# VictoriaMetrics/VictoriaLogs

Measured on NVIDIA H100. Metric: log rows scanned/sec (LogsQL phrase+regex), higher is better.
Workload: dtype u8

## Files before the change

victorialogs_b200/csrc/vl_zstd.cu:

```cuda
#include "vl_zstd.h"

#include <algorithm>
#include <array>
#include <atomic>
#include <chrono>
#include <cstdio>
#include <cstdlib>
#include <cstring>
#include <exception>
#include <thread>

#include "vl_engine.h"
#include "vl_zstd.cuh"
#include "vl_zstd_job.h"

namespace vl {

using namespace zs;

struct ZstdDev {
    DevBuf frames, blocks, bstate, huf_tab, fse_tab, huf_state, fse_state, predef, lits, seqs, frame_err, status, lists;
    bool predef_ready = false;
    cudaStream_t xstream = nullptr;
    std::vector<cudaEvent_t> events;
// ... 78 lines not shown
    auto taper = [&] { if (!group_scale_env()) m->limit_scale = (m->groups.empty() || m->n_seqs > total_seqs - total_seqs / 12) ? 1 : 4; };
    for (size_t i = 0; i < n; i++) {
        try {
            uint32_t f1 = 0, f2 = 0;
            taper();
            const size_t c1 = add_bytes_block(v[i].p, v[i].n, v[i].zoff, &info[i].lens_len, &f1);
            taper();
            const size_t c2 = add_bytes_block(v[i].p + c1, v[i].n - c1, v[i].zoff + c1, &info[i].data_len, &f2);
            if (c1 + c2 != v[i].n) throw BadInput("unexpected non-empty tail after reading bytes block with strings");
        } catch (const BadInput& e) { *bad = i; *msg = e.msg; return; }
    }
    if (!group_scale_env()) m->limit_scale = 1;
}

void ZstdJob::prepare() { m->prepare(); }

void ZstdJob::digest(uint64_t out[4]) const { m->digest(out); }

void ZstdJob::run(vlscan_ctx* ctx, const uint8_t* zsrc, uint8_t* arena) {
    Impl& J = *m;
    if (J.frames.empty()) return;
    auto now = [] { return std::chrono::duration<double>(std::chrono::steady_clock::now().time_since_epoch()).count(); };
    const double t_prep = now();
    J.prepare();
    const double t_lists = now();
    const std::vector<uint32_t>& lists = J.lists;
    if (!ctx->zdev) ctx->zdev = new ZstdDev;
    ZstdDev& D = *ctx->zdev;
    cudaStream_t st = ctx->stream;
    D.frames.ensure(J.frames.size() * sizeof(ZFrame) + 16); D.blocks.ensure(J.blocks.size() * sizeof(ZBlock) + 16); D.bstate.ensure(J.blocks.size() * sizeof(ZBlockState));
    D.frame_err.ensure(J.frames.size() * 4); D.status.ensure(16); D.lists.ensure(lists.size() * 4 + 16);
    D.huf_tab.ensure(std::max<size_t>((size_t)J.max_huf * Z_HUF_TABLE * 2, 16)); D.huf_state.ensure(std::max<size_t>((size_t)J.max_huf * sizeof(ZSlotState), 16));
    D.fse_tab.ensure(std::max<size_t>((size_t)J.max_fse * Z_FSE_SLOT_BYTES, 16)); D.fse_state.ensure(std::max<size_t>((size_t)J.max_fse * sizeof(ZSlotState), 16));
    const size_t lits_stride = (J.max_lits + 64 + 255) / 256 * 256, seqs_stride = std::max<size_t>(J.max_seqs, 1);
    D.lits.ensure(2 * lits_stride); D.seqs.ensure(2 * seqs_stride * 16);
    if (!D.xstream) VL_CUDA(cudaStreamCreateWithFlags(&D.xstream, cudaStreamNonBlocking));
    if (!D.predef_ready) {
        D.predef.ensure(Z_FSE_SLOT_BYTES);
        k_zstd_predef<<<1, 32, 0, st>>>(D.predef.as<uint8_t>());
        VL_CUDA(cudaFuncSetAttribute(k_seq_decode, cudaFuncAttributeMaxDynamicSharedMemorySize, (int)(Z_SEQ_CTA_LANES * (Z_FSE_SLOT_BYTES + Z_LINEBUF))));
        VL_CUDA(cudaFuncSetAttribute(k_huf_decode, cudaFuncAttributeMaxDynamicSharedMemorySize, (int)(Z_HUF_CTA_BLOCKS * Z_HUF_TABLE * 2)));
        ctx->launches++; VL_CUDA(cudaGetLastError());
        D.predef_ready = true;
    }
    {
        auto up16 = [](size_t n) { return (n + 15) / 16 * 16; };
        const size_t nf = up16(J.frames.size() * sizeof(ZFrame)), nb = up16(J.blocks.size() * sizeof(ZBlock)), nl = up16(lists.size() * 4);
        uint8_t* h = (uint8_t*)D.ensure_hpin(nf + nb + nl + 64);
        const double t_cp = now();
        J.spread_copy(h, J.frames.data(), J.frames.size() * sizeof(ZFrame));
        J.spread_copy(h + nf, J.blocks.data(), J.blocks.size() * sizeof(ZBlock));
        if (!lists.empty()) J.spread_copy(h + nf + nb, lists.data(), lists.size() * 4);
        if (getenv("VLSCAN_DEBUG_TIMING")) fprintf(stderr, "[vlscan zstd] host: work lists of %zu launch groups %.1f ms, %.1f MB of tables to pinned memory %.1f ms (%d threads)\n",
                                                   J.groups.size(), 1e3 * (t_lists - t_prep), (nf + nb + nl) / 1e6, 1e3 * (now() - t_cp), std::max(J.threads, 1));
        k_pull_words<<<296, 256, 0, st>>>(D.frames.as<uint4>(), (const uint4*)h, nf / 16); ctx->launches++;
        k_pull_words<<<296, 256, 0, st>>>(D.blocks.as<uint4>(), (const uint4*)(h + nf), nb / 16); ctx->launches++;
        if (nl) { k_pull_words<<<296, 256, 0, st>>>(D.lists.as<uint4>(), (const uint4*)(h + nf + nb), nl / 16); ctx->launches++; }
        VL_CUDA(cudaGetLastError());
    }
    VL_CUDA(cudaMemsetAsync(D.frame_err.p, 0, J.frames.size() * 4, st));
    VL_CUDA(cudaMemsetAsync(D.status.p, 0, 16, st));
    VL_CUDA(cudaMemsetAsync(D.bstate.p, 0, J.blocks.size() * sizeof(ZBlockState), st));
    ZView V{};
    V.src = zsrc; V.arena = arena; V.frames = D.frames.as<ZFrame>(); V.blocks = D.blocks.as<ZBlock>(); V.bstate = D.bstate.as<ZBlockState>();
    V.huf_tab = D.huf_tab.as<uint16_t>(); V.fse_tab = D.fse_tab.as<uint8_t>(); V.huf_state = D.huf_state.as<ZSlotState>(); V.fse_state = D.fse_state.as<ZSlotState>();
    V.predef = D.predef.as<uint8_t>(); V.lits = D.lits.as<uint8_t>(); V.seqs = D.seqs.as<uint4>(); V.frame_err = D.frame_err.as<unsigned int>();
    V.status = D.status.as<unsigned long long>();
    const uint32_t* L = D.lists.as<uint32_t>();
    const bool dbg = getenv("VLSCAN_DEBUG_TIMING") != nullptr;
    static const char* phase_name[6] = {"huf_build", "huf_decode", "fse_build", "seq_decode", "seq_resolve", "execute"};
    std::vector<std::pair<int, std::pair<cudaEvent_t, cudaEvent_t>>> marks;
    int phase = 0;
    static const bool overlap = [] { const char* e = getenv("VLSCAN_ZSTD_OVERLAP"); return !e || atoi(e) != 0; }();
    cudaStream_t xs = overlap ? D.xstream : st;
    cudaStream_t cur_stream = st;
    auto begin = [&](int p) { phase = p; if (dbg) { cudaEvent_t a, b; cudaEventCreate(&a); cudaEventCreate(&b); cudaEventRecord(a, cur_stream); marks.push_back({p, {a, b}}); } };
    auto launched = [&] { ctx->launches++; VL_CUDA(cudaGetLastError()); if (dbg) cudaEventRecord(marks.back().second.second, cur_stream); };
    VL_CUDA(cudaEventRecord(D.event(0), st)); VL_CUDA(cudaStreamWaitEvent(xs, D.event(0), 0));
    size_t gi = 0;
    for (const Group& g : J.groups) {
        uint32_t nh = g.huf_hi - g.huf_lo, nl = g.lit_hi - g.lit_lo, ns = g.seq_hi - g.seq_lo, nf = g.frame_hi - g.frame_lo;
        if (J.group_hook) {
            uint64_t need = 0;
            for (uint32_t i = J.frames[g.frame_lo].blk_lo; i < J.frames[g.frame_hi - 1].blk_hi; i++) need = std::max<uint64_t>(need, J.blocks[i].src + (J.blocks[i].type == ZB_RLE ? 1 : J.blocks[i].size));
            J.group_hook(need);
        }
        ZView W = V;
        W.lits = V.lits + (gi & 1) * lits_stride; W.seqs = V.seqs + (gi & 1) * seqs_stride;
        cudaEvent_t ev_entropy = D.event(1 + 2 * gi), ev_exec = D.event(2 + 2 * gi);
        cur_stream = st;
        if (gi >= 2) VL_CUDA(cudaStreamWaitEvent(st, D.event(2 + 2 * (gi - 2)), 0));
        if (nh) { begin(0); k_huf_build<<<cdiv_u(nh, 4), 128, 0, st>>>(W, L + g.huf_lo, nh); launched(); }
        if (nl) { begin(1); k_huf_decode<<<cdiv_u(nl, Z_HUF_CTA_BLOCKS), Z_HUF_CTA_BLOCKS * 4, Z_HUF_CTA_BLOCKS * Z_HUF_TABLE * 2, st>>>(W, L + g.lit_lo, nl); launched(); }
        if (ns) {
            begin(2); k_fse_build<<<cdiv_u(ns, 64), 64, 0, st>>>(W, L + g.seq_lo, ns); launched();
            begin(3); k_seq_decode<<<cdiv_u(ns, Z_SEQ_CTA_LANES), 64, Z_SEQ_CTA_LANES * (Z_FSE_SLOT_BYTES + Z_LINEBUF), st>>>(W, L + g.seq_lo, ns); launched();
        }
        VL_CUDA(cudaEventRecord(ev_entropy, st));
        VL_CUDA(cudaStreamWaitEvent(xs, ev_entropy, 0));
        cur_stream = xs;
        begin(4); k_seq_resolve<<<cdiv_u(nf, 64), 64, 0, xs>>>(W, g.frame_lo, nf); launched();
        begin(5); k_execute<<<cdiv_u((uint64_t)nf * 32, Z_EXEC_WARPS * 32), Z_EXEC_WARPS * 32, 0, xs>>>(W, L + g.ord_lo, nf); launched();
        VL_CUDA(cudaEventRecord(ev_exec, xs));
        gi++;
    }
    if (gi) VL_CUDA(cudaStreamWaitEvent(st, D.event(2 + 2 * (gi - 1)), 0));
    cur_stream = st;
    if (dbg) {
        VL_CUDA(cudaStreamSynchronize(xs)); VL_CUDA(cudaStreamSynchronize(st));
        float tot[6] = {0, 0, 0, 0, 0, 0};
        for (auto& mk : marks) { float ms = 0; cudaEventElapsedTime(&ms, mk.second.first, mk.second.second); tot[mk.first] += ms; cudaEventDestroy(mk.second.first); cudaEventDestroy(mk.second.second); }
        fprintf(stderr, "[vlscan zstd] %zu groups:", J.groups.size());
        for (int p = 0; p < 6; p++) fprintf(stderr, " %s %.2f ms", phase_name[p], tot[p]);
        fprintf(stderr, "\n");
    }
    (void)phase;
    J.ran = true;
}

void ZstdJob::check(vlscan_ctx* ctx) {
    if (!m->ran) return;
    unsigned long long stt[2] = {0, 0};
    VL_CUDA(cudaMemcpyAsync(stt, ctx->zdev->status.p, 16, cudaMemcpyDeviceToHost, ctx->stream));
    VL_CUDA(cudaStreamSynchronize(ctx->stream));
    if (!stt[0]) return;
    static const char* what[] = {"", "bad Huffman tree description", "bad Huffman stream", "bad FSE table description", "bad sequences bitstream", "match offset beyond the regenerated data",
                                 "regenerated size differs from the frame content size", "bad literals section"};
    throw BadInput(std::string("cannot decompress block: ") + (stt[0] < 8 ? what[stt[0]] : "corrupted frame") + " (frame " + std::to_string(stt[1] - 1) + " of the batch)");
}

}
```

victorialogs_b200/csrc/vl_zstd.cuh:

```cuda
#pragma once
#include <cuda_runtime.h>
#include <stdint.h>
#include "vl_zstd_types.h"

namespace vl {
namespace zs {

struct ZView {
    const uint8_t* src;
    uint8_t* arena;
    const ZFrame* frames; const ZBlock* blocks; ZBlockState* bstate;
    uint16_t* huf_tab; uint8_t* fse_tab; ZSlotState* huf_state; ZSlotState* fse_state;
    const uint8_t* predef;
    uint8_t* lits; uint4* seqs;
    unsigned int* frame_err;
    unsigned long long* status;
};

static __device__ __forceinline__ void zfail(const ZView& V, uint32_t frame, unsigned code) {
    atomicCAS(&V.frame_err[frame], 0u, code);
    atomicMax(&V.status[0], (unsigned long long)code);
    atomicMax(&V.status[1], (unsigned long long)frame + 1);
}

static __device__ __forceinline__ uint64_t ldu64(const uint8_t* p) {
    uintptr_t a = (uintptr_t)p & ~(uintptr_t)7; uint32_t sh = (uint32_t)((uintptr_t)p & 7) * 8;
    uint64_t lo = *(const uint64_t*)a;
    if (!sh) return lo;
    uint64_t hi = *(const uint64_t*)(a + 8);
    return (lo >> sh) | (hi << (64 - sh));
}
static __device__ __forceinline__ uint64_t peek64(const uint8_t* base, int64_t pos) {
    if (pos >= 64) { int junk = (int)((-pos) & 7); return ldu64(base + ((pos + 7) >> 3) - 8) << junk; }
    if (pos <= 0) return 0;
    uint64_t v = 0; int nb = (int)((pos + 7) >> 3);
    for (int i = 0; i < nb; i++) v |= (uint64_t)base[i] << (8 * i);
    return v << (64 - pos);
}
struct BackReader {
    const uint8_t* base; int64_t pos; uint64_t w; int avail;
    __device__ __forceinline__ bool init(const uint8_t* p, uint32_t len) {
        base = p; w = 0; avail = 0; pos = 0;
        if (!len) return false;
        uint32_t last = p[len - 1];
        if (!last) return false;
        pos = (int64_t)len * 8 - (int64_t)(__clz(last) - 23);
        return true;
// ... 155 lines not shown
            for (int i = 0; i < nw; i++) { if (w[i] > 11) { ok = 0; break; } if (w[i]) sum += 1u << (w[i] - 1); }
            if (ok && sum == 0) ok = 0;
            if (ok) {
                maxbits = hibit(sum) + 1;
                uint32_t left = (1u << maxbits) - sum;
                if (maxbits > 11 || (left & (left - 1)) != 0) ok = 0;
                else { w[nw++] = (uint8_t)(hibit(left) + 1); }
            }
        }
        if (ok) {
            uint32_t cnt[13]; for (int i = 0; i < 13; i++) cnt[i] = 0;
            for (int i = 0; i < nw; i++) cnt[w[i]]++;
            uint32_t nxt[13]; uint32_t acc = 0;
            for (int k = 1; k <= maxbits; k++) { nxt[k] = acc; acc += cnt[k] << (k - 1); }
            for (int i = 0; i < nw; i++) if (w[i]) { s_start[wi][i] = (uint16_t)nxt[w[i]]; nxt[w[i]] += 1u << (w[i] - 1); }
        }
        s_meta[wi][0] = nw; s_meta[wi][1] = maxbits; s_meta[wi][2] = ok;
        V.bstate[bi].huf_desc_len = desc;
    }
    __syncwarp();
    if (!s_meta[wi][2]) { if (lane == 0) zfail(V, B.frame, ZERR_HUF_DESC); return; }
    const int nw = s_meta[wi][0], maxbits = s_meta[wi][1];
    uint16_t* tab = V.huf_tab + (size_t)B.huf_own * Z_HUF_TABLE;
    for (int s = (int)lane; s < nw; s += 32) {
        uint32_t ww = w[s];
        if (!ww) continue;
        uint32_t len = 1u << (ww - 1), st = s_start[wi][s];
        uint16_t e = (uint16_t)(s | ((maxbits + 1 - ww) << 8));
        for (uint32_t k = 0; k < len; k++) tab[st + k] = e;
    }
    if (lane == 0) V.huf_state[B.huf_own].huf_maxbits = (uint8_t)maxbits;
}

static const uint32_t Z_HUF_CTA_BLOCKS = 56;
static __global__ void __launch_bounds__(Z_HUF_CTA_BLOCKS * 4) k_huf_decode(ZView V, const uint32_t* __restrict__ list, uint32_t n) {
    extern __shared__ uint16_t s_tab[];
    const uint32_t local = threadIdx.x >> 2, k = threadIdx.x & 3;
    const uint32_t first = blockIdx.x * Z_HUF_CTA_BLOCKS;
    const uint32_t here = min(Z_HUF_CTA_BLOCKS, n - first);
    for (uint32_t it = 0; it < here; it++) {
        const ZBlock& Bt = V.blocks[list[first + it]];
        const uint32_t entries = 1u << V.huf_state[Bt.huf_slot].huf_maxbits;
        const uint4* g = (const uint4*)(V.huf_tab + (size_t)Bt.huf_slot * Z_HUF_TABLE);
        uint4* d = (uint4*)(s_tab + (size_t)it * Z_HUF_TABLE);
        for (uint32_t e = threadIdx.x; e < entries / 8; e += blockDim.x) d[e] = g[e];
        if (entries < 8 && threadIdx.x == 0) d[0] = g[0];
    }
    __syncthreads();
    if (local >= here) return;
    const uint32_t bi = list[first + local];
    const ZBlock& B = V.blocks[bi];
    if (V.frame_err[B.frame]) return;
    if (B.lit_streams == 1 && k) return;
    const uint32_t maxbits = V.huf_state[B.huf_slot].huf_maxbits;
    const uint16_t* tab = s_tab + (size_t)local * Z_HUF_TABLE;
    const uint32_t desc = B.lit_type == ZL_COMPRESSED ? V.bstate[bi].huf_desc_len : 0;
    if (maxbits == 0 || desc > B.lit_comp) { zfail(V, B.frame, ZERR_HUF_STREAM); return; }
    const uint8_t* s = V.src + B.src + B.lit_hdr + desc;
    uint32_t total = B.lit_comp - desc, len, nout;
    uint8_t* out = V.lits + B.lit_off;
    if (B.lit_streams == 1) { len = total; nout = B.lit_regen; }
    else {
        if (total < 6) { if (!k) zfail(V, B.frame, ZERR_HUF_STREAM); return; }
        uint32_t s1 = s[0] | (s[1] << 8), s2 = s[2] | (s[3] << 8), s3 = s[4] | (s[5] << 8);
        if ((uint64_t)6 + s1 + s2 + s3 > total) { if (!k) zfail(V, B.frame, ZERR_HUF_STREAM); return; }
        uint32_t seg = (B.lit_regen + 3) / 4;
        if (3 * seg > B.lit_regen) { if (!k) zfail(V, B.frame, ZERR_HUF_STREAM); return; }
// ... 47 lines not shown
    if (t >= n) return;
    const uint32_t bi = list[t];
    const ZBlock& B = V.blocks[bi];
    const uint8_t* p = V.src + B.src;
    uint32_t off = B.seq_hdr + 1;
    bool ok = off <= B.size && (B.modes & 3) == 0;
    int16_t freq[53]; uint16_t nx[53];
    ZSlotState st{0, 0, 0, 0};
    for (int k = 0; k < 3 && ok; k++) {
        int mode = k == 0 ? (B.modes >> 6) & 3 : k == 1 ? (B.modes >> 4) & 3 : (B.modes >> 2) & 3;
        int max_al = k == 1 ? 8 : 9, max_syms = k == 0 ? 36 : k == 1 ? 32 : 53;
        uint32_t toff = k == 0 ? Z_FSE_LL : k == 1 ? Z_FSE_OF : Z_FSE_ML;
        int al = 0;
        if (mode == 1) {
            if (off + 1 > B.size) { ok = false; break; }
            uint32_t sym = p[off++];
            if ((int)sym >= max_syms) { ok = false; break; }
            uint8_t* slot = V.fse_tab + (size_t)B.fse_own * Z_FSE_SLOT_BYTES;
            ((uint16_t*)slot)[toff] = 0; slot[2 * Z_FSE_ENTRIES + toff] = (uint8_t)sym;
        } else if (mode == 2) {
            int ns = 0;
            uint32_t used = off < B.size ? fse_read_counts(p + off, B.size - off, max_al, max_syms, freq, &ns, &al) : 0;
            uint8_t* slot = V.fse_tab + (size_t)B.fse_own * Z_FSE_SLOT_BYTES;
            if (!used || !fse_build_seq_table((uint16_t*)slot + toff, slot + 2 * Z_FSE_ENTRIES + toff, al, freq, ns, nx)) { ok = false; break; }
            off += used;
        } else continue;
        if (k == 0) st.ll_al = (uint8_t)al; else if (k == 1) st.of_al = (uint8_t)al; else st.ml_al = (uint8_t)al;
    }
    if (!ok || off > B.size) { zfail(V, B.frame, ZERR_FSE_DESC); return; }
    if (B.fse_own != Z_PREDEF) V.fse_state[B.fse_own] = st;
    V.bstate[bi].seq_bits_off = off;
}

static const uint32_t Z_SEQ_CTA_LANES = 56;
static const uint32_t Z_LINEBUF = 272;
static const uint32_t Z_SEQ_LEAD = 160;
static __device__ __forceinline__ uint32_t lds_u32(uint32_t sa) { uint32_t v; asm volatile("ld.shared.u32 %0, [%1];" : "=r"(v) : "r"(sa)); return v; }
static __device__ __forceinline__ uint32_t bfe_u32(uint32_t a, uint32_t pos, uint32_t len) { uint32_t d; asm("bfe.u32 %0, %1, %2, %3;" : "=r"(d) : "r"(a), "r"(pos), "r"(len)); return d; }
static __device__ __forceinline__ uint32_t top_bits(uint32_t x, uint32_t n) { return __funnelshift_rc(x, 0u, 32u - n); }
struct SeqLane {
    const uint8_t* gorg;
    uint32_t ring;
    uint32_t p;
    uint32_t fc;
    const uint16_t* tr; const uint8_t* sy; const uint32_t* llv; const uint32_t* mlv;
    uint32_t sl, so, sm, r1, r2, r3, ndirty, sum_ll, sum_ml, sticky;
    uint4* out;
    __device__ __forceinline__ void fetch_chunk() {
        fc--;
        const uint32_t sa = ring + ((fc & 15u) << 4);
        const uint8_t* g = gorg + (size_t)fc * 16;
        asm volatile("cp.async.cg.shared.global [%0], [%1], 16;" ::"r"(sa), "l"(g) : "memory");
    }
    __device__ __forceinline__ void window(uint32_t& c2, uint32_t& c1, uint32_t& c0) const {
        const uint32_t k = (p - 1u) >> 5, s = (0u - p) & 31u;
        const uint32_t w3 = lds_u32(ring + ((k << 2) & 252u)), w2 = lds_u32(ring + (((k - 1u) << 2) & 252u));
        const uint32_t w1 = lds_u32(ring + (((k - 2u) << 2) & 252u)), w0 = lds_u32(ring + (((k - 3u) << 2) & 252u));
        c2 = __funnelshift_l(w2, w3, s); c1 = __funnelshift_l(w1, w2, s); c0 = __funnelshift_l(w0, w1, s);
    }
    template <bool LAST>
    __device__ __forceinline__ void step() {
        const uint32_t tl = tr[sl], to = tr[so], tm = tr[sm];
        const uint32_t oc = sy[so], vl = llv[sy[sl]], vm = mlv[sy[sm]];
        if (p < fc * 128u + Z_SEQ_LEAD * 8u && fc > 0) fetch_chunk();
        asm volatile("cp.async.commit_group;\n\tcp.async.wait_group 3;" ::: "memory");
        uint32_t c2, c1, c0;
        window(c2, c1, c0);
        const uint32_t nL = vl >> 24, nM = vm >> 24, n2 = nM + nL;
        const uint32_t ov = (1u << oc) + top_bits(c2, oc);
        const uint32_t v2 = top_bits(__funnelshift_l(c1, c2, oc), n2);
        const uint32_t ml = (vm & 0xFFFFFFu) + (v2 >> nL), ll = (vl & 0xFFFFFFu) + bfe_u32(v2, 0, nL);
        const uint32_t o3 = oc + n2;
        if (!LAST) {
            const uint32_t bL = tl >> 12, bM = tm >> 12, bO = to >> 12, n3 = bL + bM + bO;
            const bool up = o3 < 32;
            const uint32_t v3 = top_bits(__funnelshift_l(up ? c1 : c0, up ? c2 : c1, o3), n3);
            sl = Z_FSE_LL + (tl & 0xFFFu) + (v3 >> (bM + bO));
            sm = Z_FSE_ML + (tm & 0xFFFu) + bfe_u32(v3, bO, bM);
            so = Z_FSE_OF + (to & 0xFFFu) + bfe_u32(v3, 0, bO);
            p -= o3 + n3;
        } else p -= o3;
        uint32_t o;
        if (ov > 3) { o = ov - 3; r3 = r2; r2 = r1; r1 = o; }
        else {
            const uint32_t idx = ov + (ll == 0 ? 1 : 0);
            if (idx == 1) o = r1;
            else {
                o = idx == 2 ? r2 : idx == 3 ? r3 : (r1 == 0xFFFFFFFFu ? r1 : r1 - 1);
                if (idx != 2) r3 = r2;
                r2 = r1; r1 = o;
            }
        }
        ndirty += (r1 | r2 | r3) >> 31;
        *out++ = make_uint4(ll, ml, o, ov);
        sum_ll += ll; sum_ml += ml;
        sticky |= p | sum_ll | sum_ml;
    }
};
static __global__ void __launch_bounds__(64) k_seq_decode(ZView V, const uint32_t* __restrict__ list, uint32_t n) {
    extern __shared__ __align__(16) uint8_t s_fse[];
    __shared__ uint32_t s_llv[36], s_mlv[53];
    const uint32_t first = blockIdx.x * Z_SEQ_CTA_LANES;
    const uint32_t here = min(Z_SEQ_CTA_LANES, n - first);
    if (threadIdx.x < 36) s_llv[threadIdx.x] = Z_LL_BASE[threadIdx.x] | ((uint32_t)Z_LL_BITS[threadIdx.x] << 24);
    if (threadIdx.x < 53) s_mlv[threadIdx.x] = Z_ML_BASE[threadIdx.x] | ((uint32_t)Z_ML_BITS[threadIdx.x] << 24);
    for (uint32_t it = 0; it < here; it++) {
        const ZBlock& Bt = V.blocks[list[first + it]];
        const uint4* src_ll = (const uint4*)(Bt.ll_slot == Z_PREDEF ? V.predef : V.fse_tab + (size_t)Bt.ll_slot * Z_FSE_SLOT_BYTES);
        const uint4* src_ml = (const uint4*)(Bt.ml_slot == Z_PREDEF ? V.predef : V.fse_tab + (size_t)Bt.ml_slot * Z_FSE_SLOT_BYTES);
        const uint4* src_of = (const uint4*)(Bt.of_slot == Z_PREDEF ? V.predef : V.fse_tab + (size_t)Bt.of_slot * Z_FSE_SLOT_BYTES);
        uint4* d = (uint4*)(s_fse + (size_t)it * Z_FSE_SLOT_BYTES);
        for (uint32_t c = threadIdx.x; c < Z_FSE_SLOT_BYTES / 16; c += blockDim.x) {
            const uint4* src = c < 64 ? src_ll : c < 128 ? src_ml : c < 160 ? src_of : c < 192 ? src_ll : c < 224 ? src_ml : src_of;
            d[c] = src[c];
        }
    }
    __syncthreads();
    if (threadIdx.x >= here) return;
    const uint32_t bi = list[first + threadIdx.x];
    const ZBlock& B = V.blocks[bi];
    if (V.frame_err[B.frame]) return;
    const uint32_t off = V.bstate[bi].seq_bits_off;
    const int ll_al = B.ll_slot == Z_PREDEF ? 6 : V.fse_state[B.ll_slot].ll_al;
    const int of_al = B.of_slot == Z_PREDEF ? 5 : V.fse_state[B.of_slot].of_al;
    const int ml_al = B.ml_slot == Z_PREDEF ? 6 : V.fse_state[B.ml_slot].ml_al;
    if (off >= B.size) { zfail(V, B.frame, ZERR_SEQ_STREAM); return; }
    const uint64_t st = B.src + off;
    const uint32_t len = B.size - off;
    const uint32_t last = V.src[st + len - 1];
    if (!last) { zfail(V, B.frame, ZERR_SEQ_STREAM); return; }
    SeqLane L;
    const uint64_t org = (st & ~255ull) - 256;
    const uint32_t s0 = (uint32_t)(st - org) * 8;
    L.gorg = V.src + org;
    L.ring = (uint32_t)__cvta_generic_to_shared(s_fse + (size_t)Z_SEQ_CTA_LANES * Z_FSE_SLOT_BYTES + (size_t)threadIdx.x * Z_LINEBUF);
    L.p = s0 + len * 8 - (uint32_t)(__clz(last) - 23);
    L.fc = ((L.p - 1u) >> 7) + 1u;
#pragma unroll
    for (int q = 0; q < 12; q++) L.fetch_chunk();
    asm volatile("cp.async.commit_group;\n\tcp.async.wait_group 0;" ::: "memory");
    L.tr = (const uint16_t*)(s_fse + (size_t)threadIdx.x * Z_FSE_SLOT_BYTES);
    L.sy = s_fse + (size_t)threadIdx.x * Z_FSE_SLOT_BYTES + 2 * Z_FSE_ENTRIES;
    L.llv = s_llv; L.mlv = s_mlv;
    {
        uint32_t c2, c1, c0;
        L.window(c2, c1, c0);
        L.sl = Z_FSE_LL + top_bits(c2, ll_al);
        L.so = Z_FSE_OF + top_bits(__funnelshift_l(c1, c2, ll_al), of_al);
        L.sm = Z_FSE_ML + top_bits(__funnelshift_l(c1, c2, ll_al + of_al), ml_al);
        L.p -= ll_al + of_al + ml_al;
        (void)c0;
    }
    const uint32_t DIRTY = 0xFFFFFFFFu;
    L.r1 = B.rep_known ? 1 : DIRTY; L.r2 = B.rep_known ? 4 : DIRTY; L.r3 = B.rep_known ? 8 : DIRTY;
    L.ndirty = 0; L.sum_ll = 0; L.sum_ml = 0; L.sticky = L.p;
    L.out = V.seqs + B.seq_base;
    const uint32_t nseq = B.nseq;
    for (uint32_t i = 0; i + 1 < nseq; i++) L.step<false>();
    if (nseq) L.step<true>();
    asm volatile("cp.async.wait_group 0;" ::: "memory");
    if ((L.sticky >> 31) || L.p != s0 || L.sum_ll > B.lit_regen) { zfail(V, B.frame, ZERR_SEQ_STREAM); return; }
    ZBlockState& S = V.bstate[bi];
    S.out_len = B.lit_regen + L.sum_ml;
    S.clean_from = B.rep_known ? 0 : L.ndirty + 1;
    S.rep[0] = L.r1; S.rep[1] = L.r2; S.rep[2] = L.r3;
}

static __global__ void __launch_bounds__(64) k_seq_resolve(ZView V, uint32_t frame_lo, uint32_t nframes) {
    const uint32_t t = blockIdx.x * blockDim.x + threadIdx.x;
    if (t >= nframes) return;
    const uint32_t f = frame_lo + t;
    if (V.frame_err[f]) return;
    const ZFrame& F = V.frames[f];
    uint64_t out = 0;
    uint32_t r1 = 1, r2 = 4, r3 = 8;
    for (uint32_t bi = F.blk_lo; bi < F.blk_hi; bi++) {
        const ZBlock& B = V.blocks[bi];
        ZBlockState& S = V.bstate[bi];
        S.out_base = (uint32_t)out;
        if (B.type != ZB_COMPRESSED) { out += B.size; S.out_len = B.size; continue; }
        if (!B.nseq) { S.out_len = B.lit_regen; out += B.lit_regen; }
        else {
            uint4* __restrict__ sq = V.seqs + B.seq_base;
            const uint32_t redo = min(S.clean_from, B.nseq);
            for (uint32_t i = 0; i < redo; i++) {
                uint4 q = sq[i];
                uint32_t ll = q.x, ov = q.w, o;
                if (ov > 3) { o = ov - 3; r3 = r2; r2 = r1; r1 = o; }
                else {
                    uint32_t idx = ov + (ll == 0 ? 1 : 0);
                    if (idx == 1) o = r1;
                    else {
                        o = idx == 2 ? r2 : idx == 3 ? r3 : r1 - 1;
                        if (idx != 2) r3 = r2;
                        r2 = r1; r1 = o;
                    }
                }
                sq[i].z = o;
            }
            if (S.clean_from <= B.nseq) { r1 = S.rep[0]; r2 = S.rep[1]; r3 = S.rep[2]; }
            out += S.out_len;
        }
        if (out > F.fcs) { zfail(V, f, ZERR_SIZE); return; }
    }
    if (out != F.fcs) zfail(V, f, ZERR_SIZE);
}

static const uint32_t Z_RING = 4096;
static const uint32_t Z_EXEC_WARPS = 4;
static __device__ __forceinline__ uint32_t ldu32(const uint8_t* p) {
    const uintptr_t a = (uintptr_t)p & ~(uintptr_t)3;
    const uint32_t lo = *(const uint32_t*)a, hi = *(const uint32_t*)(a + 4);
    return __funnelshift_r(lo, hi, (uint32_t)((uintptr_t)p & 3) * 8);
}
static __global__ void __launch_bounds__(128) k_execute(ZView V, const uint32_t* __restrict__ order, uint32_t nframes) {
    __shared__ __align__(16) uint8_t s_ring[Z_EXEC_WARPS][Z_RING];
    const uint32_t wid = (blockIdx.x * blockDim.x + threadIdx.x) >> 5, lane = threadIdx.x & 31;
    if (wid >= nframes) return;
    const uint32_t f = order[wid];
    if (V.frame_err[f]) return;
    const ZFrame& F = V.frames[f];
    uint8_t* dst = V.arena + F.dst;
    uint8_t* ring = s_ring[threadIdx.x >> 5];
    const uint32_t abase = (uint32_t)(uintptr_t)dst;
#define VL_RIDX(p) ((abase + (p)) & (Z_RING - 1))
#define VL_RING(p) ring[VL_RIDX(p)]
    uint32_t ring_lo = 0;
    for (uint32_t bi = F.blk_lo; bi < F.blk_hi; bi++) {
        const ZBlock& B = V.blocks[bi];
        const uint32_t blk_base = V.bstate[bi].out_base;
        const uint8_t* p = V.src + B.src;
        if (B.type == ZB_RAW) { for (uint32_t k = lane; k < B.size; k += 32) { uint8_t v = p[k]; dst[blk_base + k] = v; VL_RING(blk_base + k) = v; } __syncwarp(); continue; }
        if (B.type == ZB_RLE) { uint8_t v = p[0]; for (uint32_t k = lane; k < B.size; k += 32) { dst[blk_base + k] = v; VL_RING(blk_base + k) = v; } __syncwarp(); continue; }
        const uint8_t* lit = B.lit_type == ZL_RAW ? p + B.lit_hdr : V.lits + B.lit_off;
        const bool lit_rle = B.lit_type == ZL_RLE;
        const uint8_t rle_byte = lit_rle ? p[B.lit_hdr] : 0;
        const uint4* __restrict__ sq = V.seqs + B.seq_base;
        uint32_t lit_run = 0, out_run = blk_base;
        uint4 qn = lane < B.nseq ? sq[lane] : make_uint4(0, 0, 0, 0);
        for (uint32_t g = 0; g < B.nseq; g += 32) {
            const uint4 q = qn;
            qn = g + 32 + lane < B.nseq ? sq[g + 32 + lane] : make_uint4(0, 0, 0, 0);
            uint32_t il = q.x, io = q.x + q.y;
#pragma unroll
            for (int d = 1; d < 32; d <<= 1) { uint32_t a = __shfl_up_sync(0xffffffffu, il, d), b = __shfl_up_sync(0xffffffffu, io, d); if ((int)lane >= d) { il += a; io += b; } }
            const uint32_t lit_start = il - q.x;
            const uint32_t o_start = io - q.x - q.y;
            const uint32_t T = __shfl_sync(0xffffffffu, il, 31), O = __shfl_sync(0xffffffffu, io, 31);
            const uint32_t gend = out_run + O;
            const uint32_t cnt = min(32u, B.nseq - g);
            const uint32_t ml = q.y, off = q.z, amd = out_run + o_start + q.x;
            if (__any_sync(0xffffffffu, lane < cnt && (off == 0 || off > amd))) { if (lane == 0) zfail(V, f, ZERR_OFFSET); return; }
            const uint32_t s_src = amd - off, e_src = s_src + min(ml, off);
            int dep = -1;
            {
                uint32_t lo = 0;
#pragma unroll
                for (int s = 16; s; s >>= 1) { uint32_t v = __shfl_sync(0xffffffffu, amd, (lo + s - 1) & 31); if ((lo + s - 1) < cnt && v < e_src) lo += s; }
                const uint32_t ci = (lo - 1) & 31;
                const uint32_t ca = __shfl_sync(0xffffffffu, amd, ci), cm = __shfl_sync(0xffffffffu, ml, ci);
                if (lo > 0 && ca + cm > s_src) dep = (int)lo - 1;
            }
            if (O < Z_RING) {
                uint32_t cl = (q.x + 3) >> 2, cm = (ml + 3) >> 2;
#pragma unroll
                for (int d = 1; d < 32; d <<= 1) { uint32_t a = __shfl_up_sync(0xffffffffu, cl, d), b = __shfl_up_sync(0xffffffffu, cm, d); if ((int)lane >= d) { cl += a; cm += b; } }
                const uint32_t CL = __shfl_sync(0xffffffffu, cl, 31);
                const uint32_t pk = lit_start | (o_start << 16);
                const uint8_t* lsrc = lit + lit_run;
                for (uint32_t c0 = 0; c0 < CL; c0 += 128) {
                    uint32_t w[4], at[4], nb[4];
#pragma unroll
                    for (int u = 0; u < 4; u++) {
                        nb[u] = 0; w[u] = 0; at[u] = 0;
                        if (c0 + 32 * u >= CL) continue;
// ... 124 lines not shown
```

victorialogs_b200/csrc/vl_zstd_job.h:

```cpp
#pragma once
#include <stddef.h>
#include <stdint.h>
#include <stdlib.h>
#include <string.h>
#include <algorithm>
#include <array>
#include <atomic>
#include <exception>
#include <functional>
#include <string>
#include <thread>
#include <vector>
#include "vl_zstd.h"
#include "vl_zstd_types.h"
#include "vl_zstd_walk.h"

namespace vl {

using namespace zs;

inline uint64_t group_scale_env() { static const uint64_t v = [] { const char* e = getenv("VLSCAN_ZSTD_GROUP_SCALE"); long x = e ? atol(e) : 0; return (uint64_t)(x < 0 ? 0 : x > 64 ? 64 : x); }(); return v; }
static const uint64_t kGroupLitsUnit = 512ull << 20, kGroupSeqsUnit = 64ull << 20;
static const uint32_t kGroupSlotsUnit = 32u << 10;

struct Group { uint32_t frame_lo, frame_hi; uint32_t huf_lo, huf_hi, lit_lo, lit_hi, seq_lo, seq_hi, ord_lo, ord_hi; };

struct FrameUse { uint64_t lits, seqs; uint32_t huf, fse; };

struct ZstdJobImpl {
    std::vector<ZFrame> frames;
    std::vector<ZBlock> blocks;
    std::vector<Group> groups;
    std::vector<uint32_t> lists;
    uint64_t g_lits = 0, g_seqs = 0; uint32_t g_huf = 0, g_fse = 0; uint32_t g_frame_lo = 0;
    uint64_t limit_scale = group_scale_env() ? group_scale_env() : 4;
    uint64_t max_lits = 0, max_seqs = 0; uint32_t max_huf = 0, max_fse = 0;
    uint64_t n_compressed = 0, n_seqs = 0;
    int threads = 0;
    bool prepared = false, ran = false;
    std::function<void(uint64_t)> group_hook;

    void close_group_at(uint32_t f) {
        if (g_frame_lo == f) return;
        Group g{}; g.frame_lo = g_frame_lo; g.frame_hi = f;
        groups.push_back(g);
        max_lits = std::max(max_lits, g_lits); max_seqs = std::max(max_seqs, g_seqs); max_huf = std::max(max_huf, g_huf); max_fse = std::max(max_fse, g_fse);
        g_lits = g_seqs = 0; g_huf = g_fse = 0; g_frame_lo = f;
    }
    void close_group() { close_group_at((uint32_t)frames.size()); }

    static FrameUse frame_use(const ZBlock* b, uint32_t cnt) {
        FrameUse u{0, 0, 0, 0};
        for (uint32_t i = 0; i < cnt; i++) {
            if (b[i].type != ZB_COMPRESSED) continue;
            if (b[i].lit_type >= ZL_COMPRESSED) u.lits += b[i].lit_regen;
            u.seqs += b[i].nseq; u.huf += b[i].huf_own != Z_PREDEF; u.fse += b[i].fse_own != Z_PREDEF;
        }
        return u;
    }
    FrameUse admit_frame(uint32_t f, const FrameUse& u) {
        const uint64_t m = limit_scale;
        if (g_frame_lo != f && (g_lits + u.lits > kGroupLitsUnit * m || g_seqs + u.seqs > kGroupSeqsUnit * m || g_huf + u.huf > kGroupSlotsUnit * m || g_fse + u.fse > kGroupSlotsUnit * m)) close_group_at(f);
        FrameUse base{g_lits, g_seqs, g_huf, g_fse};
        g_lits += u.lits; g_seqs += u.seqs; g_huf += u.huf; g_fse += u.fse;
        return base;
    }
    static void place_blocks(ZBlock* b, uint32_t cnt, FrameUse base, uint64_t& n_compressed, uint64_t& n_seqs) {
        for (uint32_t i = 0; i < cnt; i++) {
            ZBlock& B = b[i];
            if (B.type != ZB_COMPRESSED) continue;
// ... 85 lines not shown
        const size_t G = groups.size();
        std::vector<std::vector<uint32_t>> gl(G);
        std::vector<std::array<uint32_t, 4>> cnt(G);
        std::atomic<size_t> next{0};
        const int T = (int)std::max<size_t>(1, std::min<size_t>((size_t)std::max(threads, 1), G));
        on_threads(T, [&](int) {
            std::vector<std::pair<uint32_t, uint32_t>> v; std::vector<uint32_t> count;
            for (;;) {
                const size_t gi = next.fetch_add(1);
                if (gi >= G) return;
                const Group& g = groups[gi];
                std::vector<uint32_t>& L = gl[gi];
                const uint32_t blo = frames[g.frame_lo].blk_lo, bhi = frames[g.frame_hi - 1].blk_hi;
                auto by_desc = [&] {
                    uint32_t kmax = 0; for (auto& e : v) kmax = std::max(kmax, e.first);
                    if (v.size() >= 64 && kmax < (1u << 16)) {
                        count.assign((size_t)kmax + 2, 0);
                        for (auto& e : v) count[kmax - e.first + 1]++;
                        for (uint32_t k = 0; k <= kmax; k++) count[k + 1] += count[k];
                        const size_t at = L.size(); L.resize(at + v.size());
                        for (auto& e : v) L[at + count[kmax - e.first]++] = e.second;
                    } else {
                        std::stable_sort(v.begin(), v.end(), [](const auto& a, const auto& b) { return a.first > b.first; });
                        for (auto& e : v) L.push_back(e.second);
                    }
                    v.clear();
                };
                for (uint32_t i = blo; i < bhi; i++) if (blocks[i].type == ZB_COMPRESSED && blocks[i].lit_type == ZL_COMPRESSED) L.push_back(i);
                cnt[gi][0] = (uint32_t)L.size();
                for (uint32_t i = blo; i < bhi; i++) if (blocks[i].type == ZB_COMPRESSED && blocks[i].lit_type >= ZL_COMPRESSED) v.push_back({blocks[i].lit_regen >> 9, i});
                by_desc(); cnt[gi][1] = (uint32_t)L.size();
                for (uint32_t i = blo; i < bhi; i++) if (blocks[i].type == ZB_COMPRESSED && blocks[i].nseq) v.push_back({blocks[i].nseq >> 6, i});
                by_desc(); cnt[gi][2] = (uint32_t)L.size();
                for (uint32_t i = g.frame_lo; i < g.frame_hi; i++) v.push_back({(uint32_t)(frames[i].fcs >> 10), i});
                by_desc(); cnt[gi][3] = (uint32_t)L.size();
            }
        });
        size_t total = 0; for (auto& L : gl) total += L.size();
        if (total > 0xFFFFFFF0ull) throw BadInput("too many ZSTD blocks in one batch");
        lists.resize(total);
        size_t off = 0;
        for (size_t gi = 0; gi < G; gi++) {
            Group& g = groups[gi];
            g.huf_lo = (uint32_t)off; g.huf_hi = g.lit_lo = (uint32_t)(off + cnt[gi][0]); g.lit_hi = g.seq_lo = (uint32_t)(off + cnt[gi][1]);
            g.seq_hi = g.ord_lo = (uint32_t)(off + cnt[gi][2]); g.ord_hi = (uint32_t)(off + cnt[gi][3]);
            if (!gl[gi].empty()) memcpy(lists.data() + off, gl[gi].data(), gl[gi].size() * 4);
            off += gl[gi].size();
        }
    }

    void spread_copy(void* dst, const void* src, size_t n) const {
        const int T = (int)std::max<size_t>(1, std::min<size_t>((size_t)std::max(threads, 1), n / (4u << 20) + 1));
        on_threads(T, [&](int t) { const size_t lo = n * (size_t)t / (size_t)T, hi = n * (size_t)(t + 1) / (size_t)T; if (hi > lo) memcpy((uint8_t*)dst + lo, (const uint8_t*)src + lo, hi - lo); });
    }

    void digest(uint64_t out[4]) const {
        const ZstdJobImpl& J = *this;
        auto mix = [](uint64_t& h, uint64_t v) { h = (h ^ v) * 0x9E3779B97F4A7C15ull; h ^= h >> 29; };
        uint64_t h0 = 1, h1 = 2, h2 = 3, h3 = 4;
        for (const ZFrame& f : J.frames) { mix(h0, f.dst); mix(h0, f.fcs); mix(h0, ((uint64_t)f.blk_lo << 32) | f.blk_hi); }
        for (const ZBlock& b : J.blocks) {
            mix(h1, b.src); mix(h1, b.lit_off); mix(h1, b.seq_base); mix(h1, ((uint64_t)b.size << 32) | b.frame); mix(h1, ((uint64_t)b.lit_hdr << 32) | b.lit_regen);
            mix(h1, ((uint64_t)b.lit_comp << 32) | b.nseq); mix(h1, ((uint64_t)b.seq_hdr << 32) | b.huf_slot); mix(h1, ((uint64_t)b.huf_own << 32) | b.fse_own);
            mix(h1, ((uint64_t)b.ll_slot << 32) | b.of_slot); mix(h1, ((uint64_t)b.ml_slot << 32) | ((uint64_t)b.type << 24) | ((uint64_t)b.lit_type << 16) | ((uint64_t)b.lit_streams << 8) | b.modes); mix(h1, b.rep_known);
        }
        for (const Group& g : J.groups) for (uint32_t x : {g.frame_lo, g.frame_hi, g.huf_lo, g.huf_hi, g.lit_lo, g.lit_hi, g.seq_lo, g.seq_hi, g.ord_lo, g.ord_hi}) mix(h2, x);
        for (uint64_t x : {J.max_lits, J.max_seqs, (uint64_t)J.max_huf, (uint64_t)J.max_fse, J.n_compressed, J.n_seqs, (uint64_t)J.groups.size()}) mix(h2, x);
        for (uint32_t x : J.lists) mix(h3, x);
        out[0] = h0; out[1] = h1; out[2] = h2; out[3] = h3;
    }
};

}
```

victorialogs_b200/csrc/vl_zstd_types.h:

```cpp
#pragma once
#include <stdint.h>

namespace vl {
namespace zs {

enum { ZERR_NONE = 0, ZERR_HUF_DESC = 1, ZERR_HUF_STREAM = 2, ZERR_FSE_DESC = 3, ZERR_SEQ_STREAM = 4, ZERR_OFFSET = 5, ZERR_SIZE = 6, ZERR_LITERALS = 7 };
enum { ZB_RAW = 0, ZB_RLE = 1, ZB_COMPRESSED = 2 };
enum { ZL_RAW = 0, ZL_RLE = 1, ZL_COMPRESSED = 2, ZL_TREELESS = 3 };
static const uint32_t Z_PREDEF = 0xFFFFFFFFu;
static const uint32_t Z_HUF_TABLE = 2048;
static const uint32_t Z_FSE_LL = 0, Z_FSE_ML = 512, Z_FSE_OF = 1024, Z_FSE_ENTRIES = 1280, Z_FSE_SLOT_BYTES = 3 * 1280;

struct ZFrame {
    uint64_t dst;
    uint64_t fcs;
    uint32_t blk_lo, blk_hi;
};
struct ZBlock {
    uint64_t src;
    uint64_t lit_off;
    uint64_t seq_base;
    uint32_t size;
    uint32_t frame;
    uint32_t lit_hdr;
    uint32_t lit_regen, lit_comp;
    uint32_t nseq;
    uint32_t seq_hdr;
    uint32_t huf_slot;
    uint32_t huf_own;
    uint32_t fse_own;
    uint32_t ll_slot, of_slot, ml_slot;
    uint8_t type, lit_type, lit_streams, modes;
    uint8_t rep_known;
    uint8_t pad[3];
};
struct ZBlockState {
    uint32_t huf_desc_len;
    uint32_t seq_bits_off;
    uint32_t out_len;
    uint32_t out_base;
    uint32_t clean_from;
    uint32_t rep[3];
};
struct ZSlotState { uint8_t huf_maxbits, ll_al, of_al, ml_al; };
// ... 4 lines not shown
```

Measured before the change: 21.35 billion.

## Pack decoded zstd sequences into 64-bit words and shrink seq/huf CTA sizes

Decoded sequences are stored as packed 64-bit words (18-bit literal and match lengths, a 2-bit repeat code, a 26-bit offset) whenever every frame in a launch group fits the offset limit. A templated wide uint4 path remains as the fallback. This halves the sequence buffer traffic between seq_decode, seq_resolve and execute. Separately, Huffman and sequence CTA sizes drop from 56 to 28 lanes, block size becomes a rounded-up warp multiple, and execute gets a max-shared-memory carveout hint. The packed path risks subtle bugs if length fields exceed 18 bits.

```diff
diff --git a/victorialogs_b200/csrc/vl_zstd.cu b/victorialogs_b200/csrc/vl_zstd.cu
--- a/victorialogs_b200/csrc/vl_zstd.cu
+++ b/victorialogs_b200/csrc/vl_zstd.cu
@@ -134,14 +134,17 @@
     D.frame_err.ensure(J.frames.size() * 4); D.status.ensure(16); D.lists.ensure(lists.size() * 4 + 16);
     D.huf_tab.ensure(std::max<size_t>((size_t)J.max_huf * Z_HUF_TABLE * 2, 16)); D.huf_state.ensure(std::max<size_t>((size_t)J.max_huf * sizeof(ZSlotState), 16));
     D.fse_tab.ensure(std::max<size_t>((size_t)J.max_fse * Z_FSE_SLOT_BYTES, 16)); D.fse_state.ensure(std::max<size_t>((size_t)J.max_fse * sizeof(ZSlotState), 16));
-    const size_t lits_stride = (J.max_lits + 64 + 255) / 256 * 256, seqs_stride = std::max<size_t>(J.max_seqs, 1);
-    D.lits.ensure(2 * lits_stride); D.seqs.ensure(2 * seqs_stride * 16);
+    const size_t lits_stride = (J.max_lits + 64 + 255) / 256 * 256, seqs_stride = std::max<size_t>(J.max_seqs, 1) * (J.any_wide_seqs ? 16 : 8);
+    D.lits.ensure(2 * lits_stride); D.seqs.ensure(2 * seqs_stride);
     if (!D.xstream) VL_CUDA(cudaStreamCreateWithFlags(&D.xstream, cudaStreamNonBlocking));
     if (!D.predef_ready) {
         D.predef.ensure(Z_FSE_SLOT_BYTES);
         k_zstd_predef<<<1, 32, 0, st>>>(D.predef.as<uint8_t>());
-        VL_CUDA(cudaFuncSetAttribute(k_seq_decode, cudaFuncAttributeMaxDynamicSharedMemorySize, (int)(Z_SEQ_CTA_LANES * (Z_FSE_SLOT_BYTES + Z_LINEBUF))));
+        VL_CUDA(cudaFuncSetAttribute(k_seq_decode<SeqPacked>, cudaFuncAttributeMaxDynamicSharedMemorySize, (int)(Z_SEQ_CTA_LANES * (Z_FSE_SLOT_BYTES + Z_LINEBUF))));
+        VL_CUDA(cudaFuncSetAttribute(k_seq_decode<SeqWide>, cudaFuncAttributeMaxDynamicSharedMemorySize, (int)(Z_SEQ_CTA_LANES * (Z_FSE_SLOT_BYTES + Z_LINEBUF))));
         VL_CUDA(cudaFuncSetAttribute(k_huf_decode, cudaFuncAttributeMaxDynamicSharedMemorySize, (int)(Z_HUF_CTA_BLOCKS * Z_HUF_TABLE * 2)));
+        VL_CUDA(cudaFuncSetAttribute(k_execute<SeqPacked>, cudaFuncAttributePreferredSharedMemoryCarveout, (int)cudaSharedmemCarveoutMaxShared));
+        VL_CUDA(cudaFuncSetAttribute(k_execute<SeqWide>, cudaFuncAttributePreferredSharedMemoryCarveout, (int)cudaSharedmemCarveoutMaxShared));
         ctx->launches++; VL_CUDA(cudaGetLastError());
         D.predef_ready = true;
     }
@@ -166,7 +169,7 @@
     ZView V{};
     V.src = zsrc; V.arena = arena; V.frames = D.frames.as<ZFrame>(); V.blocks = D.blocks.as<ZBlock>(); V.bstate = D.bstate.as<ZBlockState>();
     V.huf_tab = D.huf_tab.as<uint16_t>(); V.fse_tab = D.fse_tab.as<uint8_t>(); V.huf_state = D.huf_state.as<ZSlotState>(); V.fse_state = D.fse_state.as<ZSlotState>();
-    V.predef = D.predef.as<uint8_t>(); V.lits = D.lits.as<uint8_t>(); V.seqs = D.seqs.as<uint4>(); V.frame_err = D.frame_err.as<unsigned int>();
+    V.predef = D.predef.as<uint8_t>(); V.lits = D.lits.as<uint8_t>(); V.seqs = D.seqs.as<uint8_t>(); V.frame_err = D.frame_err.as<unsigned int>();
     V.status = D.status.as<unsigned long long>();
     const uint32_t* L = D.lists.as<uint32_t>();
     const bool dbg = getenv("VLSCAN_DEBUG_TIMING") != nullptr;
@@ -188,7 +191,7 @@
             J.group_hook(need);
         }
         ZView W = V;
-        W.lits = V.lits + (gi & 1) * lits_stride; W.seqs = V.seqs + (gi & 1) * seqs_stride;
+        W.lits = V.lits + (gi & 1) * lits_stride; W.seqs = (uint8_t*)V.seqs + (gi & 1) * seqs_stride;
         cudaEvent_t ev_entropy = D.event(1 + 2 * gi), ev_exec = D.event(2 + 2 * gi);
         cur_stream = st;
         if (gi >= 2) VL_CUDA(cudaStreamWaitEvent(st, D.event(2 + 2 * (gi - 2)), 0));
@@ -196,13 +199,23 @@
         if (nl) { begin(1); k_huf_decode<<<cdiv_u(nl, Z_HUF_CTA_BLOCKS), Z_HUF_CTA_BLOCKS * 4, Z_HUF_CTA_BLOCKS * Z_HUF_TABLE * 2, st>>>(W, L + g.lit_lo, nl); launched(); }
         if (ns) {
             begin(2); k_fse_build<<<cdiv_u(ns, 64), 64, 0, st>>>(W, L + g.seq_lo, ns); launched();
-            begin(3); k_seq_decode<<<cdiv_u(ns, Z_SEQ_CTA_LANES), 64, Z_SEQ_CTA_LANES * (Z_FSE_SLOT_BYTES + Z_LINEBUF), st>>>(W, L + g.seq_lo, ns); launched();
+            const size_t smem = Z_SEQ_CTA_LANES * (Z_FSE_SLOT_BYTES + Z_LINEBUF);
+            begin(3);
+            if (g.wide_seqs) k_seq_decode<SeqWide><<<cdiv_u(ns, Z_SEQ_CTA_LANES), Z_SEQ_CTA_THREADS, smem, st>>>(W, L + g.seq_lo, ns);
+            else k_seq_decode<SeqPacked><<<cdiv_u(ns, Z_SEQ_CTA_LANES), Z_SEQ_CTA_THREADS, smem, st>>>(W, L + g.seq_lo, ns);
+            launched();
         }
         VL_CUDA(cudaEventRecord(ev_entropy, st));
         VL_CUDA(cudaStreamWaitEvent(xs, ev_entropy, 0));
         cur_stream = xs;
-        begin(4); k_seq_resolve<<<cdiv_u(nf, 64), 64, 0, xs>>>(W, g.frame_lo, nf); launched();
-        begin(5); k_execute<<<cdiv_u((uint64_t)nf * 32, Z_EXEC_WARPS * 32), Z_EXEC_WARPS * 32, 0, xs>>>(W, L + g.ord_lo, nf); launched();
+        begin(4);
+        if (g.wide_seqs) k_seq_resolve<SeqWide><<<cdiv_u(nf, 64), 64, 0, xs>>>(W, g.frame_lo, nf);
+        else k_seq_resolve<SeqPacked><<<cdiv_u(nf, 64), 64, 0, xs>>>(W, g.frame_lo, nf);
+        launched();
+        begin(5);
+        if (g.wide_seqs) k_execute<SeqWide><<<cdiv_u((uint64_t)nf * 32, Z_EXEC_WARPS * 32), Z_EXEC_WARPS * 32, 0, xs>>>(W, L + g.ord_lo, nf);
+        else k_execute<SeqPacked><<<cdiv_u((uint64_t)nf * 32, Z_EXEC_WARPS * 32), Z_EXEC_WARPS * 32, 0, xs>>>(W, L + g.ord_lo, nf);
+        launched();
         VL_CUDA(cudaEventRecord(ev_exec, xs));
         gi++;
     }
diff --git a/victorialogs_b200/csrc/vl_zstd.cuh b/victorialogs_b200/csrc/vl_zstd.cuh
--- a/victorialogs_b200/csrc/vl_zstd.cuh
+++ b/victorialogs_b200/csrc/vl_zstd.cuh
@@ -12,7 +12,7 @@
     const ZFrame* frames; const ZBlock* blocks; ZBlockState* bstate;
     uint16_t* huf_tab; uint8_t* fse_tab; ZSlotState* huf_state; ZSlotState* fse_state;
     const uint8_t* predef;
-    uint8_t* lits; uint4* seqs;
+    uint8_t* lits; void* seqs;
     unsigned int* frame_err;
     unsigned long long* status;
 };
@@ -234,7 +234,10 @@
     if (lane == 0) V.huf_state[B.huf_own].huf_maxbits = (uint8_t)maxbits;
 }
 
-static const uint32_t Z_HUF_CTA_BLOCKS = 56;
+#ifndef VL_ZSTD_HUF_CTA_BLOCKS
+#define VL_ZSTD_HUF_CTA_BLOCKS 28
+#endif
+static const uint32_t Z_HUF_CTA_BLOCKS = VL_ZSTD_HUF_CTA_BLOCKS;
 static __global__ void __launch_bounds__(Z_HUF_CTA_BLOCKS * 4) k_huf_decode(ZView V, const uint32_t* __restrict__ list, uint32_t n) {
     extern __shared__ uint16_t s_tab[];
     const uint32_t local = threadIdx.x >> 2, k = threadIdx.x & 3;
@@ -348,12 +351,35 @@
     V.bstate[bi].seq_bits_off = off;
 }
 
-static const uint32_t Z_SEQ_CTA_LANES = 56;
+#ifndef VL_ZSTD_SEQ_CTA_LANES
+#define VL_ZSTD_SEQ_CTA_LANES 28
+#endif
+static const uint32_t Z_SEQ_CTA_LANES = VL_ZSTD_SEQ_CTA_LANES;
+static const uint32_t Z_SEQ_CTA_THREADS = (Z_SEQ_CTA_LANES + 31) / 32 * 32;
 static const uint32_t Z_LINEBUF = 272;
 static const uint32_t Z_SEQ_LEAD = 160;
+struct SeqWide {
+    typedef uint4 T;
+    static __device__ __forceinline__ T pack(uint32_t ll, uint32_t ml, uint32_t o, uint32_t ov) { return make_uint4(ll, ml, o, ov); }
+    static __device__ __forceinline__ uint4 unpack(const T& q) { return make_uint4(q.x, q.y, q.z, 0); }
+    static __device__ __forceinline__ uint32_t ll(const T& q) { return q.x; }
+    static __device__ __forceinline__ uint32_t offset_value(const T& q) { return q.w; }
+    static __device__ __forceinline__ void set_offset(T& dst, const T&, uint32_t o) { dst.z = o; }
+};
+struct SeqPacked {
+    typedef unsigned long long T;
+    static __device__ __forceinline__ T pack(uint32_t ll, uint32_t ml, uint32_t o, uint32_t ov) {
+        return (T)ll | ((T)ml << 18) | ((T)(ov <= 3 ? ov : 0) << 36) | ((T)min(o, Z_PACKED_OFF_MAX) << 38);
+    }
+    static __device__ __forceinline__ uint4 unpack(const T& q) { return make_uint4((uint32_t)q & 0x3FFFFu, (uint32_t)(q >> 18) & 0x3FFFFu, (uint32_t)(q >> 38), 0); }
+    static __device__ __forceinline__ uint32_t ll(const T& q) { return (uint32_t)q & 0x3FFFFu; }
+    static __device__ __forceinline__ uint32_t offset_value(const T& q) { const uint32_t c = (uint32_t)(q >> 36) & 3u; return c ? c : (uint32_t)(q >> 38) + 3u; }
+    static __device__ __forceinline__ void set_offset(T& dst, const T& q, uint32_t o) { dst = (q & ((1ull << 38) - 1)) | ((T)min(o, Z_PACKED_OFF_MAX) << 38); }
+};
 static __device__ __forceinline__ uint32_t lds_u32(uint32_t sa) { uint32_t v; asm volatile("ld.shared.u32 %0, [%1];" : "=r"(v) : "r"(sa)); return v; }
 static __device__ __forceinline__ uint32_t bfe_u32(uint32_t a, uint32_t pos, uint32_t len) { uint32_t d; asm("bfe.u32 %0, %1, %2, %3;" : "=r"(d) : "r"(a), "r"(pos), "r"(len)); return d; }
 static __device__ __forceinline__ uint32_t top_bits(uint32_t x, uint32_t n) { return __funnelshift_rc(x, 0u, 32u - n); }
+template <class R>
 struct SeqLane {
     const uint8_t* gorg;
     uint32_t ring;
@@ -361,7 +387,7 @@
     uint32_t fc;
     const uint16_t* tr; const uint8_t* sy; const uint32_t* llv; const uint32_t* mlv;
     uint32_t sl, so, sm, r1, r2, r3, ndirty, sum_ll, sum_ml, sticky;
-    uint4* out;
+    typename R::T* out;
     __device__ __forceinline__ void fetch_chunk() {
         fc--;
         const uint32_t sa = ring + ((fc & 15u) << 4);
@@ -408,18 +434,19 @@
             }
         }
         ndirty += (r1 | r2 | r3) >> 31;
-        *out++ = make_uint4(ll, ml, o, ov);
+        *out++ = R::pack(ll, ml, o, ov);
         sum_ll += ll; sum_ml += ml;
         sticky |= p | sum_ll | sum_ml;
     }
 };
-static __global__ void __launch_bounds__(64) k_seq_decode(ZView V, const uint32_t* __restrict__ list, uint32_t n) {
+template <class R>
+static __global__ void __launch_bounds__(Z_SEQ_CTA_THREADS) k_seq_decode(ZView V, const uint32_t* __restrict__ list, uint32_t n) {
     extern __shared__ __align__(16) uint8_t s_fse[];
     __shared__ uint32_t s_llv[36], s_mlv[53];
     const uint32_t first = blockIdx.x * Z_SEQ_CTA_LANES;
     const uint32_t here = min(Z_SEQ_CTA_LANES, n - first);
-    if (threadIdx.x < 36) s_llv[threadIdx.x] = Z_LL_BASE[threadIdx.x] | ((uint32_t)Z_LL_BITS[threadIdx.x] << 24);
-    if (threadIdx.x < 53) s_mlv[threadIdx.x] = Z_ML_BASE[threadIdx.x] | ((uint32_t)Z_ML_BITS[threadIdx.x] << 24);
+    for (uint32_t c = threadIdx.x; c < 36; c += blockDim.x) s_llv[c] = Z_LL_BASE[c] | ((uint32_t)Z_LL_BITS[c] << 24);
+    for (uint32_t c = threadIdx.x; c < 53; c += blockDim.x) s_mlv[c] = Z_ML_BASE[c] | ((uint32_t)Z_ML_BITS[c] << 24);
     for (uint32_t it = 0; it < here; it++) {
         const ZBlock& Bt = V.blocks[list[first + it]];
         const uint4* src_ll = (const uint4*)(Bt.ll_slot == Z_PREDEF ? V.predef : V.fse_tab + (size_t)Bt.ll_slot * Z_FSE_SLOT_BYTES);
@@ -445,7 +472,7 @@
     const uint32_t len = B.size - off;
     const uint32_t last = V.src[st + len - 1];
     if (!last) { zfail(V, B.frame, ZERR_SEQ_STREAM); return; }
-    SeqLane L;
+    SeqLane<R> L;
     const uint64_t org = (st & ~255ull) - 256;
     const uint32_t s0 = (uint32_t)(st - org) * 8;
     L.gorg = V.src + org;
@@ -470,10 +497,10 @@
     const uint32_t DIRTY = 0xFFFFFFFFu;
     L.r1 = B.rep_known ? 1 : DIRTY; L.r2 = B.rep_known ? 4 : DIRTY; L.r3 = B.rep_known ? 8 : DIRTY;
     L.ndirty = 0; L.sum_ll = 0; L.sum_ml = 0; L.sticky = L.p;
-    L.out = V.seqs + B.seq_base;
+    L.out = (typename R::T*)V.seqs + B.seq_base;
     const uint32_t nseq = B.nseq;
-    for (uint32_t i = 0; i + 1 < nseq; i++) L.step<false>();
-    if (nseq) L.step<true>();
+    for (uint32_t i = 0; i + 1 < nseq; i++) L.template step<false>();
+    if (nseq) L.template step<true>();
     asm volatile("cp.async.wait_group 0;" ::: "memory");
     if ((L.sticky >> 31) || L.p != s0 || L.sum_ll > B.lit_regen) { zfail(V, B.frame, ZERR_SEQ_STREAM); return; }
     ZBlockState& S = V.bstate[bi];
@@ -482,6 +509,7 @@
     S.rep[0] = L.r1; S.rep[1] = L.r2; S.rep[2] = L.r3;
 }
 
+template <class R>
 static __global__ void __launch_bounds__(64) k_seq_resolve(ZView V, uint32_t frame_lo, uint32_t nframes) {
     const uint32_t t = blockIdx.x * blockDim.x + threadIdx.x;
     if (t >= nframes) return;
@@ -497,11 +525,11 @@
         if (B.type != ZB_COMPRESSED) { out += B.size; S.out_len = B.size; continue; }
         if (!B.nseq) { S.out_len = B.lit_regen; out += B.lit_regen; }
         else {
-            uint4* __restrict__ sq = V.seqs + B.seq_base;
+            typename R::T* __restrict__ sq = (typename R::T*)V.seqs + B.seq_base;
             const uint32_t redo = min(S.clean_from, B.nseq);
             for (uint32_t i = 0; i < redo; i++) {
-                uint4 q = sq[i];
-                uint32_t ll = q.x, ov = q.w, o;
+                const typename R::T q = sq[i];
+                uint32_t ll = R::ll(q), ov = R::offset_value(q), o;
                 if (ov > 3) { o = ov - 3; r3 = r2; r2 = r1; r1 = o; }
                 else {
                     uint32_t idx = ov + (ll == 0 ? 1 : 0);
@@ -512,7 +540,7 @@
                         r2 = r1; r1 = o;
                     }
                 }
-                sq[i].z = o;
+                R::set_offset(sq[i], q, o);
             }
             if (S.clean_from <= B.nseq) { r1 = S.rep[0]; r2 = S.rep[1]; r3 = S.rep[2]; }
             out += S.out_len;
@@ -522,14 +550,21 @@
     if (out != F.fcs) zfail(V, f, ZERR_SIZE);
 }
 
-static const uint32_t Z_RING = 4096;
-static const uint32_t Z_EXEC_WARPS = 4;
+#ifndef VL_ZSTD_RING
+#define VL_ZSTD_RING 4096
+#endif
+#ifndef VL_ZSTD_EXEC_WARPS
+#define VL_ZSTD_EXEC_WARPS 4
+#endif
+static const uint32_t Z_RING = VL_ZSTD_RING;
+static const uint32_t Z_EXEC_WARPS = VL_ZSTD_EXEC_WARPS;
 static __device__ __forceinline__ uint32_t ldu32(const uint8_t* p) {
     const uintptr_t a = (uintptr_t)p & ~(uintptr_t)3;
     const uint32_t lo = *(const uint32_t*)a, hi = *(const uint32_t*)(a + 4);
     return __funnelshift_r(lo, hi, (uint32_t)((uintptr_t)p & 3) * 8);
 }
-static __global__ void __launch_bounds__(128) k_execute(ZView V, const uint32_t* __restrict__ order, uint32_t nframes) {
+template <class R>
+static __global__ void __launch_bounds__(Z_EXEC_WARPS * 32) k_execute(ZView V, const uint32_t* __restrict__ order, uint32_t nframes) {
     __shared__ __align__(16) uint8_t s_ring[Z_EXEC_WARPS][Z_RING];
     const uint32_t wid = (blockIdx.x * blockDim.x + threadIdx.x) >> 5, lane = threadIdx.x & 31;
     if (wid >= nframes) return;
@@ -551,12 +586,12 @@
         const uint8_t* lit = B.lit_type == ZL_RAW ? p + B.lit_hdr : V.lits + B.lit_off;
         const bool lit_rle = B.lit_type == ZL_RLE;
         const uint8_t rle_byte = lit_rle ? p[B.lit_hdr] : 0;
-        const uint4* __restrict__ sq = V.seqs + B.seq_base;
+        const typename R::T* __restrict__ sq = (const typename R::T*)V.seqs + B.seq_base;
         uint32_t lit_run = 0, out_run = blk_base;
-        uint4 qn = lane < B.nseq ? sq[lane] : make_uint4(0, 0, 0, 0);
+        typename R::T qn = lane < B.nseq ? sq[lane] : typename R::T{};
         for (uint32_t g = 0; g < B.nseq; g += 32) {
-            const uint4 q = qn;
-            qn = g + 32 + lane < B.nseq ? sq[g + 32 + lane] : make_uint4(0, 0, 0, 0);
+            const uint4 q = R::unpack(qn);
+            qn = g + 32 + lane < B.nseq ? sq[g + 32 + lane] : typename R::T{};
             uint32_t il = q.x, io = q.x + q.y;
 #pragma unroll
             for (int d = 1; d < 32; d <<= 1) { uint32_t a = __shfl_up_sync(0xffffffffu, il, d), b = __shfl_up_sync(0xffffffffu, io, d); if ((int)lane >= d) { il += a; io += b; } }
diff --git a/victorialogs_b200/csrc/vl_zstd_job.h b/victorialogs_b200/csrc/vl_zstd_job.h
--- a/victorialogs_b200/csrc/vl_zstd_job.h
+++ b/victorialogs_b200/csrc/vl_zstd_job.h
@@ -23,7 +23,10 @@
 static const uint64_t kGroupLitsUnit = 512ull << 20, kGroupSeqsUnit = 64ull << 20;
 static const uint32_t kGroupSlotsUnit = 32u << 10;
 
-struct Group { uint32_t frame_lo, frame_hi; uint32_t huf_lo, huf_hi, lit_lo, lit_hi, seq_lo, seq_hi, ord_lo, ord_hi; };
+struct Group {
+    uint32_t frame_lo, frame_hi; uint32_t huf_lo, huf_hi, lit_lo, lit_hi, seq_lo, seq_hi, ord_lo, ord_hi;
+    bool wide_seqs;
+};
 
 struct FrameUse { uint64_t lits, seqs; uint32_t huf, fse; };
 
@@ -36,6 +39,7 @@
     uint64_t limit_scale = group_scale_env() ? group_scale_env() : 4;
     uint64_t max_lits = 0, max_seqs = 0; uint32_t max_huf = 0, max_fse = 0;
     uint64_t n_compressed = 0, n_seqs = 0;
+    bool any_wide_seqs = false;
     int threads = 0;
     bool prepared = false, ran = false;
     std::function<void(uint64_t)> group_hook;
@@ -187,8 +191,10 @@
                 by_desc(); cnt[gi][1] = (uint32_t)L.size();
                 for (uint32_t i = blo; i < bhi; i++) if (blocks[i].type == ZB_COMPRESSED && blocks[i].nseq) v.push_back({blocks[i].nseq >> 6, i});
                 by_desc(); cnt[gi][2] = (uint32_t)L.size();
-                for (uint32_t i = g.frame_lo; i < g.frame_hi; i++) v.push_back({(uint32_t)(frames[i].fcs >> 10), i});
+                bool wide = false;
+                for (uint32_t i = g.frame_lo; i < g.frame_hi; i++) { v.push_back({(uint32_t)(frames[i].fcs >> 10), i}); wide |= frames[i].fcs > Z_PACKED_OFF_MAX; }
                 by_desc(); cnt[gi][3] = (uint32_t)L.size();
+                groups[gi].wide_seqs = wide;
             }
         });
         size_t total = 0; for (auto& L : gl) total += L.size();
@@ -200,6 +206,7 @@
             g.huf_lo = (uint32_t)off; g.huf_hi = g.lit_lo = (uint32_t)(off + cnt[gi][0]); g.lit_hi = g.seq_lo = (uint32_t)(off + cnt[gi][1]);
             g.seq_hi = g.ord_lo = (uint32_t)(off + cnt[gi][2]); g.ord_hi = (uint32_t)(off + cnt[gi][3]);
             if (!gl[gi].empty()) memcpy(lists.data() + off, gl[gi].data(), gl[gi].size() * 4);
+            any_wide_seqs |= g.wide_seqs;
             off += gl[gi].size();
         }
     }
diff --git a/victorialogs_b200/csrc/vl_zstd_types.h b/victorialogs_b200/csrc/vl_zstd_types.h
--- a/victorialogs_b200/csrc/vl_zstd_types.h
+++ b/victorialogs_b200/csrc/vl_zstd_types.h
@@ -10,6 +10,7 @@
 static const uint32_t Z_PREDEF = 0xFFFFFFFFu;
 static const uint32_t Z_HUF_TABLE = 2048;
 static const uint32_t Z_FSE_LL = 0, Z_FSE_ML = 512, Z_FSE_OF = 1024, Z_FSE_ENTRIES = 1280, Z_FSE_SLOT_BYTES = 3 * 1280;
+static const uint32_t Z_PACKED_OFF_MAX = (1u << 26) - 1;
 
 struct ZFrame {
     uint64_t dst;
```

Result: no change. 21.37 billion (median of 6 runs) (+0.1%).
